# Corv/CUDA-GMM-MPI

Hardware: AMD Instinct MI355X
Metric: em_iterations_per_sec (higher is better)
Workload: dtype bf16; 1 GPU; model=gmm_em, n_events=1000000, events_per_gpu=1000000, dims=24, clusters=64, parallelism=dp1, device=cuda

## Files before the change

### cuda_gmm_mpi_amd/engine.py

```python
from __future__ import annotations

import dataclasses

import numpy as np
import torch

from .models.merge import HostClusters, reduce_order_batched
from .models.seed import seed_means_host, seed_state
from .models.state import GmmState
from .ops import functional as F
from .parallel import dist as pdist
from .utils.config import GmmConfig, em_epsilon, rissanen_score
from .utils.timers import Profile


@dataclasses.dataclass
class SweepResult:
    state: GmmState
    num_clusters: int
    min_rissanen: float
    likelihood: float
    rissanen_by_k: dict[int, float]


# ... 132 lines not shown
        st = self.state.shrink(k)
        empty_f = torch.empty(0, dtype=torch.float32, device=self.device)
        empty_b = torch.empty(0, dtype=torch.bfloat16, device=self.device)
        logdet = torch.empty(k, dtype=torch.float32, device=self.device)
        hip_ext().constants(st.R.contiguous(), st.means.contiguous(),
                            empty_f, st.Rinv, logdet, empty_f, empty_f,
                            empty_b, empty_f, False)

    def _sync_add(self, k: int) -> None:
        if self._add is not None:
            st = self.state.shrink(k)
            self._add[:k] = st.constant + torch.log(st.pi)


    def _estep(self, k: int, need_lik: bool = True) -> torch.Tensor | None:
        st = self.state.shrink(k)
        with self.profile.time("e_step"):
            self._w_is_logw = False
            if self.use_fused_estep and self.use_lds_estep:
                add = self._add[:k]
                if self.mfac32 is not None:
                    w, lik = F.estep_fused_f32_lds(self.x_estep,
                                                   self.mfac32[:k], add,
                                                   self.w[:k], need_lik)
                else:
                    w, lik = F.estep_fused_lds(self.x_estep, self.mfac[:k],
                                               add, self.w[:k], need_lik)
            elif self.use_fused_estep:
                self._w_is_logw = True
                add = self._add[:k]
                if self.mfac32 is not None:
                    w, lik = F.estep_fused_f32(self.x_estep, self.mfac32[:k],
                                               add, self.w[:k], self._lse,
                                               need_lik)
                else:
                    w, lik = F.estep_fused(self.x_estep, self.mfac[:k], add,
                                           self.w[:k], self._lse, need_lik)
            elif self.use_big_estep:
                add = self._add[:k]
                if self.mfac32 is not None:
                    logw = F.estep_logw_big_f32(self.x_estep,
                                                self.mfac32[:k], add,
                                                self.w[:k])
                    self._w_is_logw = True
                else:
                    logw = F.estep_logw_big(self.x_estep, self.mfac[:k],
                                            add, self.w[:k])
                lik = F.estep_lse(logw, self._lse, need_lik)
                self._w_is_logw = True
            elif self.device.type == "cuda":
                logw = F.estep_logw(
                    self.x_estep, st.means, st.Rinv, st.constant, st.pi,
                    self.cfg.diag_only, out=self.w[:k],
                )
                lik = F.estep_lse(logw, self._lse, need_lik)
                self._w_is_logw = True
            else:
                logw = F.estep_logw(
                    self.x_estep, st.means, st.Rinv, st.constant, st.pi,
                    self.cfg.diag_only, out=self.w[:k],
                )
                w, lik = F.estep_posteriors(logw)
        self.profile.count("regroup")
        return lik

    def _finish_likelihood(self, lik_part: torch.Tensor) -> None:
        with self.profile.time("comm"):
            t = lik_part.reshape(1)
            pdist.all_reduce_(t)
            self._lik_dev.copy_(t)

    def _reduce_likelihood(self, lik_part: torch.Tensor) -> float:
        self._finish_likelihood(lik_part)
        return float(self._lik_dev.item())

    def _iteration_body(self, k: int, need_lik: bool = True) -> None:
        self._mstep(k)
        lik = self._estep(k, need_lik)
        if need_lik and lik is not None:
            self._finish_likelihood(lik)

    def _can_graph(self) -> bool:
        import os
        if not self.use_graphs or os.environ.get("GMM_NO_GRAPHS"):
            return False
        if self.device.type != "cuda":
            return False
        if self.world > 1:
            return bool(os.environ.get("GMM_DIST_GRAPHS"))
        return True

    def _mstep(self, k: int) -> None:
        st = self.state.shrink(k)
# ... 378 lines not shown
```

### cuda_gmm_mpi_amd/ops/functional.py

```python
from __future__ import annotations

import os

import torch

from . import cpu_reference as cpu
from .backend import hip_ext


def estep_logw(x: torch.Tensor, means: torch.Tensor, rinv: torch.Tensor,
               constant: torch.Tensor, pi: torch.Tensor,
               diag_only: bool = False,
               out: torch.Tensor | None = None) -> torch.Tensor:
    if x.is_cuda:
        k, n = means.shape[0], x.shape[1]
        if out is None:
            out = torch.empty((k, n), dtype=torch.float32, device=x.device)
        hip_ext().estep_logw(
            x, means, rinv, constant, torch.log(pi), out, bool(diag_only)
        )
        return out
    logw = cpu.estep_logw(x.float(), means, rinv, constant, pi, diag_only)
    if out is not None:
        out.copy_(logw)
        return out
    return logw


def estep_posteriors(logw: torch.Tensor) -> tuple[torch.Tensor, torch.Tensor]:
    if logw.is_cuda:
        nblocks = 1024
        partial = torch.zeros(nblocks, dtype=torch.float32, device=logw.device)
        hip_ext().estep_posteriors(logw, partial)
        return logw, partial.sum()
    w, lik = cpu.estep_posteriors(logw)
    logw.copy_(w)
    return logw, lik


def estep_lse(logw: torch.Tensor, lse: torch.Tensor,
              need_lik: bool = True) -> torch.Tensor | None:
    nblocks = 1024
    partial = torch.zeros(nblocks, dtype=torch.float32, device=logw.device)
    hip_ext().estep_lse(logw, lse, partial)
    if not need_lik:
        return None
    lik = torch.empty(1, dtype=torch.float32, device=logw.device)
    hip_ext().reduce_scalar(partial, lik)
    return lik


def mstep_n_means(x_aug_t: torch.Tensor, w: torch.Tensor
                  ) -> tuple[torch.Tensor, torch.Tensor]:
    nm = w @ x_aug_t
    return nm[:, -1].contiguous(), nm[:, :-1].contiguous()


_tri_cache: dict = {}


def _tri_unpack_index(d: int, device) -> torch.Tensor:
    key = (d, str(device))
    idx = _tri_cache.get(key)
    if idx is None:
        full = torch.empty(d, d, dtype=torch.long)
        for i in range(d):
            for j in range(d):
                r, c = (i, j) if i >= j else (j, i)
                full[i, j] = r * (r + 1) // 2 + c
        idx = full.reshape(-1).to(device)
# ... 93 lines not shown
                if out is not None:
                    const_t.copy_(cval)
                else:
                    const_t = cval
                add_t.copy_(cval + torch.log(pi_t))
            return rinv, const_t
        hip_ext().constants(r, means, empty, rinv, logdet, empty, empty,
                            mfac, mfac32, bool(diag_only))
        const = -d * 0.5 * cpu.LOG_2PI - 0.5 * logdet
        if out is not None:
            out[1].copy_(const)
            const = out[1]
        return rinv, const
    rinv_c, const_c = cpu.compute_constants(r, diag_only)
    if out is not None:
        out[0].copy_(rinv_c)
        out[1].copy_(const_c)
        return out[0], out[1]
    return rinv_c, const_c


def _run_fused(entry: str, tile: int, z: torch.Tensor, fac: torch.Tensor,
               add: torch.Tensor, w_out: torch.Tensor, need_lik: bool,
               *lse: torch.Tensor) -> tuple[torch.Tensor, torch.Tensor | None]:
    ext = hip_ext()
    nblk = (z.shape[1] + tile - 1) // tile
    partial = torch.empty(nblk, dtype=torch.float32, device=z.device)
    getattr(ext, entry)(z, fac, add, w_out, *lse, partial)
    if not need_lik:
        return w_out, None
    lik = torch.empty(1, dtype=torch.float32, device=z.device)
    ext.reduce_scalar(partial, lik)
    return w_out, lik


def estep_fused(z: torch.Tensor, mfac: torch.Tensor, add: torch.Tensor,
                w_out: torch.Tensor, lse: torch.Tensor,
                need_lik: bool = True
                ) -> tuple[torch.Tensor, torch.Tensor | None]:
    return _run_fused("estep_fused", 256, z, mfac, add, w_out, need_lik, lse)


def estep_fused_available(device: torch.device, dtype: str, d: int,
                          k: int) -> bool:
    return device.type == "cuda" and d <= 31


def estep_fused_lds_available(device: torch.device, dtype: str, d: int,
                              k: int) -> bool:
    if device.type != "cuda" or d > 31:
        return False
    if dtype == "bf16":
        return 128 * 40 * 2 + 4 * k * 132 <= 64 * 1024
    return 4 * (128 * 33 + k * 132) <= 64 * 1024


def estep_fused_lds(z: torch.Tensor, mfac: torch.Tensor, add: torch.Tensor,
                    w_out: torch.Tensor, need_lik: bool = True
                    ) -> tuple[torch.Tensor, torch.Tensor | None]:
    legacy = os.environ.get("GMM_ESTEP_LDS", "lds2") == "legacy"
    return _run_fused("estep_fused_lds" if legacy else "estep_fused_lds2",
                      128, z, mfac, add, w_out, need_lik)


def estep_fused_f32_lds(z: torch.Tensor, mfac32: torch.Tensor,
                        add: torch.Tensor, w_out: torch.Tensor,
                        need_lik: bool = True
                        ) -> tuple[torch.Tensor, torch.Tensor | None]:
    return _run_fused("estep_fused_f32_lds", 128, z, mfac32, add, w_out,
                      need_lik)


def estep_fused_f32(z: torch.Tensor, mfac32: torch.Tensor, add: torch.Tensor,
                    w_out: torch.Tensor, lse: torch.Tensor,
                    need_lik: bool = True
                    ) -> tuple[torch.Tensor, torch.Tensor | None]:
    return _run_fused("estep_fused_f32", 256, z, mfac32, add, w_out,
                      need_lik, lse)


def estep_big_available(device: torch.device, dtype: str, d: int) -> bool:
    return device.type == "cuda" and dtype in ("bf16", "fp32") and 1 <= d <= 142


def mfac_shape(d: int) -> tuple[int, int, int]:
    rows = ((d + 31) // 32) * 32
    kc = (d + 1 + 15) // 16
    kct = 2 if kc <= 2 else 3 if kc == 3 else 5 if kc <= 5 else 9
    return 2, rows, kct * 16


def estep_logw_big(z: torch.Tensor, mfac: torch.Tensor, add: torch.Tensor,
                   out: torch.Tensor) -> torch.Tensor:
    hip_ext().estep_logw_big(z, mfac, add, out)
    return out


def estep_logw_big_f32(z: torch.Tensor, mfac32: torch.Tensor,
                       add: torch.Tensor, out: torch.Tensor) -> torch.Tensor:
    hip_ext().estep_logw_big_f32(z, mfac32, add, out)
    return out
# ... 92 lines not shown
```

### cuda_gmm_mpi_amd/ops/hip/estep_fused.hip

```cpp
#pragma once

#include "gmm_common.h"

namespace gmm {

struct FacB16 {
  using In = __hip_bfloat16;
  using Z = __bf16;
  static constexpr int ZROW = 40;
  static constexpr int CELLS = 2 * 32 * 32;

  bf16x8 h0, l0, h1, l1;
  float add;

  __device__ __forceinline__ void load(const In* mfac, const float* addv,
                                       int c, int j32, int g2) {
    const bf16x8* mf = (const bf16x8*)mfac;
    const int64_t base = ((int64_t)c * 2) * 32 * 4;
    h0 = mf[base + j32 * 4 + g2];
    l0 = mf[base + 32 * 4 + j32 * 4 + g2];
    h1 = mf[base + j32 * 4 + 2 + g2];
    l1 = mf[base + 32 * 4 + j32 * 4 + 2 + g2];
    add = addv[c];
  }
};

struct FacF32 {
  using In = float;
  using Z = float;
  static constexpr int ZROW = 33;
  static constexpr int CELLS = 32 * 32;
};

template <typename Fac, int BE>
constexpr int z_tile_floats() {
  return BE * Fac::ZROW * (int)sizeof(typename Fac::Z) / 4;
}

__device__ __forceinline__ float sqnorm(const f32x16_t& y) {
  float s = 0.0f;
#pragma unroll
  for (int r = 0; r < 16; ++r) s = fmaf(y[r], y[r], s);
  return s;
}

constexpr int EST_BE = 256;

template <typename Fac>
constexpr size_t est_lds_bytes() {
  return sizeof(float) *
         (z_tile_floats<Fac, EST_BE>() + (2 * (NT / WAVE) + 1) * EST_BE);
}

__global__ void __launch_bounds__(NT)
estep_fused_kernel(const __hip_bfloat16* __restrict__ z,
                   const __hip_bfloat16* __restrict__ mfac,
                   const float* __restrict__ add,
                   float* __restrict__ w_out, float* __restrict__ lse_out,
                   float* __restrict__ partial, int d, int k, int64_t n) {
  extern __shared__ float lds[];
  __hip_bfloat16* zs = (__hip_bfloat16*)lds;
  float* mstate = lds + (EST_BE * FacB16::ZROW) / 2;
  float* sstate = mstate + (NT / WAVE) * EST_BE;
  float* lse = sstate + (NT / WAVE) * EST_BE;

// ... 446 lines not shown
    const int t = threadIdx.x;
    float m = lw[t];
#pragma unroll 4
    for (int c = 1; c < k; ++c) m = fmaxf(m, lw[c * lrow + t]);
    float s = 0.0f;
#pragma unroll 4
    for (int c = 0; c < k; ++c) {
      const float e = __expf(lw[c * lrow + t] - m);
      lw[c * lrow + t] = e;
      s += e;
    }
    const float inv = 1.0f / s;
#pragma unroll 4
    for (int c = 0; c < k; ++c)
      w_out[(int64_t)c * n + e0 + t] = lw[c * lrow + t] * inv;
    acc = m + __logf(s);
  }
  __shared__ float wsum[NT / WAVE];
  block_sum(acc, wsum, partial);
}

constexpr int ESTL2_NS = 8;

__global__ void __launch_bounds__(NT, 3)
estep_fused_lds2_kernel(const __hip_bfloat16* __restrict__ z,
                        const __hip_bfloat16* __restrict__ mfac,
                        const float* __restrict__ add,
                        float* __restrict__ w_out,
                        float* __restrict__ partial, int d, int k, int64_t n,
                        int vec4) {
  extern __shared__ float lds[];
  constexpr int lrow = ESTL_LROW;
  constexpr int ZROW = FacB16::ZROW;
  __hip_bfloat16* zs = (__hip_bfloat16*)lds;
  float* lw = lds + z_tile_floats<FacB16, ESTL_BE>();

  const int wave = __builtin_amdgcn_readfirstlane(threadIdx.x / WAVE);
  const int lane = threadIdx.x & (WAVE - 1);
  const int64_t e0 = (int64_t)blockIdx.x * ESTL_BE;
  const int cnt = (int)min((int64_t)ESTL_BE, n - e0);

  {
    const unsigned short* zu = (const unsigned short*)z;
    const int e = threadIdx.x & (ESTL_BE - 1);
    const int o_lo = wave >> 1;
    unsigned short v[2][8];
// ... 40 lines not shown
  bf16x8 b0[ESTL_BE / 32], b1[ESTL_BE / 32];
#pragma unroll
  for (int t = 0; t < ESTL_BE / 32; ++t) {
    b0[t] = *(const bf16x8*)(zs + (t * 32 + j32) * ZROW + 8 * g2);
    b1[t] = *(const bf16x8*)(zs + (t * 32 + j32) * ZROW + 16 + 8 * g2);
  }
  auto cluster = [&](const FacB16& f, int c) {
    f32x16_t y[ESTL_BE / 32];
#pragma unroll
    for (int t = 0; t < ESTL_BE / 32; ++t)
      y[t] = __builtin_amdgcn_mfma_f32_32x32x16_bf16(
          f.h0, b0[t], (f32x16_t)(0.0f), 0, 0, 0);
#pragma unroll
    for (int t = 0; t < ESTL_BE / 32; ++t)
      y[t] = __builtin_amdgcn_mfma_f32_32x32x16_bf16(f.h1, b1[t], y[t], 0, 0, 0);
#pragma unroll
    for (int t = 0; t < ESTL_BE / 32; ++t)
      y[t] = __builtin_amdgcn_mfma_f32_32x32x16_bf16(f.l0, b0[t], y[t], 0, 0, 0);
#pragma unroll
    for (int t = 0; t < ESTL_BE / 32; ++t)
      y[t] = __builtin_amdgcn_mfma_f32_32x32x16_bf16(f.l1, b1[t], y[t], 0, 0, 0);
    float s[ESTL_BE / 32];
#pragma unroll
    for (int t = 0; t < ESTL_BE / 32; ++t) s[t] = sqnorm(y[t]);
#pragma unroll
    for (int t = 0; t < ESTL_BE / 32; t += 2) {
      const auto sw = __builtin_amdgcn_permlane32_swap(
          __float_as_uint(s[t]), __float_as_uint(s[t + 1]), false, false);
      const float st = __uint_as_float(sw[0]) + __uint_as_float(sw[1]);
      lw[c * lrow + (t + g2) * 32 + j32] = -0.5f * st + f.add;
    }
  };
  FacB16 fa, fb;
  int c = wave;
  fa.load(mfac, add, min(c, k - 1), j32, g2);
  for (; c + nwaves < k; c += 2 * nwaves) {
    fb.load(mfac, add, c + nwaves, j32, g2);
    __builtin_amdgcn_sched_barrier(0);
    cluster(fa, c);
    __builtin_amdgcn_sched_barrier(0);
    fa.load(mfac, add, min(c + 2 * nwaves, k - 1), j32, g2);
    __builtin_amdgcn_sched_barrier(0);
    cluster(fb, c + nwaves);
    __builtin_amdgcn_sched_barrier(0);
  }
  if (c < k) cluster(fa, c);
  __syncthreads();
// ... 90 lines not shown
```

### cuda_gmm_mpi_amd/ops/hip/gmm_ext.hip

```cpp
#include <ATen/hip/HIPContext.h>
#include <torch/extension.h>

#include <hip/hip_runtime.h>
#include <hip/hip_bf16.h>

#define HIP_CHECK(expr)                                                     \
  do {                                                                      \
    hipError_t _e = (expr);                                                 \
    TORCH_CHECK(_e == hipSuccess, "HIP error: ", hipGetErrorString(_e));    \
  } while (0)

#include "gmm_kernels.hip"

namespace {

constexpr int kNT = 256;

hipStream_t stream() { return at::hip::getCurrentHIPStream().stream(); }

void check_f32(const torch::Tensor& t, const char* name) {
  TORCH_CHECK(t.is_cuda() && t.is_contiguous() &&
                  t.scalar_type() == torch::kFloat32,
              name, " must be contiguous fp32 on device");
}
// ... 138 lines not shown
  else if (ppt <= 4) LAUNCH_COV(4);
  else if (ppt <= 8) LAUNCH_COV(8);
  else if (ppt <= 17) LAUNCH_COV(17);
  else if (ppt <= 33) LAUNCH_COV(33);
  else TORCH_CHECK(false, "D too large for covariance kernel (max 128)");
#undef LAUNCH_COV
  HIP_CHECK(hipGetLastError());
}

void mstep_covariance_partials(torch::Tensor x, torch::Tensor w,
                               torch::Tensor lse, torch::Tensor partials) {
  TORCH_CHECK(x.is_cuda() && x.is_contiguous(), "x must be contiguous device");
  check_f32(w, "w");
  check_f32(partials, "partials");
  if (x.scalar_type() == torch::kFloat32) {
    mstep_cov_impl<float>(x, w, lse, partials);
  } else if (x.scalar_type() == torch::kBFloat16) {
    mstep_cov_impl<__hip_bfloat16>(x, w, lse, partials);
  } else {
    TORCH_CHECK(false, "x must be fp32 or bf16");
  }
}

void constants(torch::Tensor r, torch::Tensor means, torch::Tensor pi,
               torch::Tensor rinv, torch::Tensor logdet,
               torch::Tensor constant, torch::Tensor add, torch::Tensor mfac,
               torch::Tensor mfac32, bool diag_only) {
  check_f32(r, "r");
  check_f32(means, "means");
  check_f32(rinv, "rinv");
  check_f32(logdet, "logdet");
  const int k = (int)r.size(0);
  const int d = (int)r.size(1);
  const bool make_mfac = mfac.numel() > 0;
  __hip_bfloat16* mp = nullptr;
  float* mp32 = nullptr;
  if (mfac32.numel() > 0) {
    TORCH_CHECK(mfac32.is_cuda() && mfac32.is_contiguous() &&
                    mfac32.scalar_type() == torch::kFloat32,
                "mfac32 must be contiguous fp32");
    mp32 = mfac32.data_ptr<float>();
  }
  if (make_mfac) {
    const int rows = gmm::mfac_rows(d);
    const int kct = gmm::mfac_kct(d);
    TORCH_CHECK(mfac.is_cuda() && mfac.is_contiguous() &&
                    mfac.scalar_type() == torch::kBFloat16 &&
                    mfac.numel() == (int64_t)k * 2 * rows * kct * 16 &&
                    d <= 142,
                "mfac must be bf16 [K,2,RT*32,KCT*16] with D <= 142");
    mp = reinterpret_cast<__hip_bfloat16*>(mfac.data_ptr());
  }
  auto s = stream();
  float* pip = pi.numel() > 0 ? pi.data_ptr<float>() : nullptr;
  float* cst = constant.numel() > 0 ? constant.data_ptr<float>() : nullptr;
  float* addp = add.numel() > 0 ? add.data_ptr<float>() : nullptr;
  TORCH_CHECK(addp == nullptr || pip != nullptr, "add output requires pi");
  if (diag_only) {
    hipLaunchKernelGGL(gmm::constants_diag_kernel, dim3(k), dim3(kNT), 0, s,
                       r.data_ptr<float>(), rinv.data_ptr<float>(),
                       logdet.data_ptr<float>(), d);
    if (make_mfac) {
      hipLaunchKernelGGL(gmm::emit_mfac_from_r_kernel, dim3(k), dim3(kNT),
                         sizeof(float) * (2 * (size_t)d * (d | 1) + d), s,
                         r.data_ptr<float>(), means.data_ptr<float>(), mp,
                         mp32, d, nullptr, nullptr, nullptr);
    }
  } else {
    const size_t lds = sizeof(float) * (2 * (size_t)d * (d | 1) + d);
    if (lds > 64 * 1024) {
      HIP_CHECK(hipFuncSetAttribute(
          reinterpret_cast<const void*>(&gmm::constants_lu_kernel),
          hipFuncAttributeMaxDynamicSharedMemorySize, (int)lds));
    }
// ... 225 lines not shown
void estep_fused_lds(torch::Tensor z, torch::Tensor mfac, torch::Tensor add,
                     torch::Tensor w_out, torch::Tensor partial) {
  launch_fused_lds<gmm::FacB16>("estep_fused_lds",
                                gmm::estep_fused_lds_kernel, z, mfac, add,
                                w_out, partial);
}

void estep_fused_f32_lds(torch::Tensor z, torch::Tensor mfac32,
                         torch::Tensor add, torch::Tensor w_out,
                         torch::Tensor partial) {
  launch_fused_lds<gmm::FacF32>("estep_fused_f32_lds",
                                gmm::estep_fused_f32_lds_kernel, z, mfac32,
                                add, w_out, partial);
}

void estep_fused_lds2(torch::Tensor z, torch::Tensor mfac, torch::Tensor add,
                      torch::Tensor w_out, torch::Tensor partial) {
  const char* name = "estep_fused_lds2";
  const FusedShape s = check_fused<gmm::FacB16>(name, z, mfac, add, w_out,
                                                partial, gmm::ESTL_BE);
  const int vec4 = s.n % 4 == 0 &&
                   reinterpret_cast<uintptr_t>(w_out.data_ptr()) % 16 == 0;
  const size_t lds = fused_lds_budget<gmm::FacB16>(name, s.k);
  hipLaunchKernelGGL(gmm::estep_fused_lds2_kernel, dim3((uint32_t)s.nblk),
                     dim3(kNT), lds, stream(), data_as<__hip_bfloat16>(z),
                     data_as<__hip_bfloat16>(mfac), add.data_ptr<float>(),
                     w_out.data_ptr<float>(), partial.data_ptr<float>(), s.d,
                     s.k, s.n, vec4);
  HIP_CHECK(hipGetLastError());
}

void estep_logw_big(torch::Tensor z, torch::Tensor mfac, torch::Tensor add,
                    torch::Tensor logw) {
  TORCH_CHECK(z.is_cuda() && z.is_contiguous() &&
                  z.scalar_type() == torch::kBFloat16,
              "z must be contiguous bf16 [D,N]");
  TORCH_CHECK(mfac.is_contiguous() && mfac.scalar_type() == torch::kBFloat16);
  check_f32(add, "add");
  check_f32(logw, "logw");
  const int d = (int)z.size(0);
  const int64_t n = z.size(1);
  const int k = (int)add.size(0);
  TORCH_CHECK(d >= 1 && d <= 142, "estep_logw_big supports D <= 143");
  TORCH_CHECK(logw.size(0) == k && logw.size(1) == n, "logw shape");
  const int kct = gmm::mfac_kct(d);
  const int rows = gmm::mfac_rows(d);
  const int rt_n = rows / 32;
  const int arow = kct * 16 + 8;
  const size_t lds256 = (size_t)(2 * rows + 256) * arow * 2 +
                        (size_t)rt_n * 256 * 4;
  const size_t lds128 = (size_t)(2 * rows + 128) * arow * 2 +
// ... 103 lines not shown
                     stream(), x.data_ptr<float>(), w.data_ptr<float>(),
                     lse_ptr(lse, n), partials.data_ptr<float>(), d, k, n,
                     nchunk);
  HIP_CHECK(hipGetLastError());
}

void mfma_probe32(torch::Tensor a, torch::Tensor b, torch::Tensor c) {
  TORCH_CHECK(a.scalar_type() == torch::kBFloat16 && a.numel() == 32 * 16);
  TORCH_CHECK(b.scalar_type() == torch::kBFloat16 && b.numel() == 16 * 32);
  check_f32(c, "c");
  hipLaunchKernelGGL(gmm::mfma_probe32_kernel, dim3(1), dim3(64), 0, stream(),
                     reinterpret_cast<const __hip_bfloat16*>(a.data_ptr()),
                     reinterpret_cast<const __hip_bfloat16*>(b.data_ptr()),
                     c.data_ptr<float>());
  HIP_CHECK(hipGetLastError());
}

void reduce_chunks(torch::Tensor partials, torch::Tensor out) {
  check_f32(partials, "partials");
  check_f32(out, "out");
  const int c = (int)partials.size(0);
  const int64_t m = partials.numel() / c;
  TORCH_CHECK(out.numel() == m, "out shape");
  const int grid = (int)std::min<int64_t>((m + kNT - 1) / kNT, 4096);
  hipLaunchKernelGGL(gmm::reduce_chunks_kernel, dim3(grid), dim3(kNT), 0,
                     stream(), partials.data_ptr<float>(),
                     out.data_ptr<float>(), c, m);
  HIP_CHECK(hipGetLastError());
}

void reduce_scalar(torch::Tensor in, torch::Tensor out) {
  check_f32(in, "in");
  check_f32(out, "out");
  TORCH_CHECK(out.numel() >= 1);
  hipLaunchKernelGGL(gmm::reduce_scalar_kernel, dim3(1), dim3(kNT), 0,
                     stream(), in.data_ptr<float>(), out.data_ptr<float>(),
                     in.numel());
  HIP_CHECK(hipGetLastError());
}

void mstep_finalize(torch::Tensor packed, torch::Tensor avgvar,
                    int64_t world, torch::Tensor n_out, torch::Tensor means,
                    torch::Tensor r_out, torch::Tensor pi, bool diag_only) {
  check_f32(packed, "packed");
  check_f32(avgvar, "avgvar");
  check_f32(n_out, "n_out");
  check_f32(means, "means");
  check_f32(r_out, "r_out");
// ... 20 lines not shown
                         torch::Tensor mfac32) {
  check_f32(packed, "packed");
  check_f32(avgvar, "avgvar");
  check_f32(n_out, "n_out");
  check_f32(means, "means");
  check_f32(r_out, "r_out");
  check_f32(pi, "pi");
  check_f32(constant, "constant");
  check_f32(add, "add");
  const int k = (int)means.size(0);
  const int d = (int)means.size(1);
  TORCH_CHECK(packed.size(0) == k &&
                  packed.size(1) == (d + 1) * (d + 2) / 2,
              "packed shape mismatch");
  TORCH_CHECK(mfac.numel() > 0 && mfac.scalar_type() == torch::kBFloat16 &&
              mfac.is_contiguous());
  __hip_bfloat16* mp =
      reinterpret_cast<__hip_bfloat16*>(mfac.data_ptr());
  float* mp32 = nullptr;
  if (mfac32.numel() > 0) {
    check_f32(mfac32, "mfac32");
    mp32 = mfac32.data_ptr<float>();
  }
  const size_t lds = sizeof(float) * (2 * (size_t)d * (d | 1) + d);
  if (lds > 64 * 1024) {
    HIP_CHECK(hipFuncSetAttribute(
        reinterpret_cast<const void*>(&gmm::mstep_finalize_emit_kernel),
        hipFuncAttributeMaxDynamicSharedMemorySize, (int)lds));
  }
  hipLaunchKernelGGL(gmm::mstep_finalize_emit_kernel, dim3(k), dim3(kNT),
                     lds, stream(), packed.data_ptr<float>(),
                     avgvar.data_ptr<float>(), (int)world,
                     n_out.data_ptr<float>(), means.data_ptr<float>(),
                     r_out.data_ptr<float>(), pi.data_ptr<float>(),
                     constant.data_ptr<float>(), add.data_ptr<float>(), mp,
                     mp32, d, k);
  HIP_CHECK(hipGetLastError());
}

void emit_factors(torch::Tensor r, torch::Tensor means,
                  torch::Tensor mfac, torch::Tensor mfac32,
                  torch::Tensor pi, torch::Tensor constant,
                  torch::Tensor add) {
  check_f32(r, "r");
  check_f32(means, "means");
  const int k = (int)r.size(0);
  const int d = (int)r.size(1);
  __hip_bfloat16* mp = nullptr;
  float* mp32 = nullptr;
  if (mfac.numel() > 0) {
    TORCH_CHECK(mfac.scalar_type() == torch::kBFloat16 && mfac.is_contiguous());
    mp = reinterpret_cast<__hip_bfloat16*>(mfac.data_ptr());
  }
  if (mfac32.numel() > 0) {
    check_f32(mfac32, "mfac32");
    mp32 = mfac32.data_ptr<float>();
  }
  const size_t lds = sizeof(float) * (2 * (size_t)d * (d | 1) + d);
  if (lds > 64 * 1024) {
    HIP_CHECK(hipFuncSetAttribute(
        reinterpret_cast<const void*>(&gmm::emit_mfac_from_r_kernel),
        hipFuncAttributeMaxDynamicSharedMemorySize, (int)lds));
  }
  const float* pip = pi.numel() > 0 ? pi.data_ptr<float>() : nullptr;
  float* cst = constant.numel() > 0 ? constant.data_ptr<float>() : nullptr;
  float* addp = add.numel() > 0 ? add.data_ptr<float>() : nullptr;
  TORCH_CHECK(addp == nullptr || pip != nullptr, "add output requires pi");
  hipLaunchKernelGGL(gmm::emit_mfac_from_r_kernel, dim3(k), dim3(kNT),
                     lds, stream(), r.data_ptr<float>(),
                     means.data_ptr<float>(), mp, mp32, d, pip, cst, addp);
  HIP_CHECK(hipGetLastError());
}

void mfma_probe(torch::Tensor a, torch::Tensor b, torch::Tensor c) {
  TORCH_CHECK(a.scalar_type() == torch::kBFloat16 && a.numel() == 16 * 32);
  TORCH_CHECK(b.scalar_type() == torch::kBFloat16 && b.numel() == 32 * 16);
  check_f32(c, "c");
  hipLaunchKernelGGL(gmm::mfma_probe_kernel, dim3(1), dim3(64), 0, stream(),
                     reinterpret_cast<const __hip_bfloat16*>(a.data_ptr()),
                     reinterpret_cast<const __hip_bfloat16*>(b.data_ptr()),
// ... 56 lines not shown
```

### cuda_gmm_mpi_amd/ops/hip/gmm_kernels.hip

```cpp
#include "gmm_common.h"

namespace gmm {

__device__ inline void tri_row_col(int t, int* i, int* j) {
  int r = (int)((sqrtf(8.0f * t + 1.0f) - 1.0f) * 0.5f);
  while ((r + 1) * (r + 2) / 2 <= t) ++r;
  while (r * (r + 1) / 2 > t) --r;
  *i = r;
  *j = t - r * (r + 1) / 2;
}

__device__ inline int mfma_b16_k(int group, int u) { return 8 * group + u; }

__host__ __device__ inline int kc_tier(int kc) {
  return kc <= 2 ? 2 : kc == 3 ? 3 : kc <= 5 ? 5 : 9;
}

__host__ __device__ inline int mfac_rows(int d) { return ((d + 31) / 32) * 32; }
__host__ __device__ inline int mfac_kct(int d) {
  return kc_tier((d + 1 + 15) / 16);
}

__device__ inline void stage_cluster_params(
    const float* __restrict__ means, const float* __restrict__ rinv,
// ... 152 lines not shown
    float s = 0.0f;
#pragma unroll 4
    for (int c = 0; c < k; ++c) s += __expf(logw[(int64_t)c * n + e] - m);
    const float denom = m + __logf(s);
    lse[e] = denom;
    acc += denom;
  }
  __shared__ float wsum[NT / WAVE];
  for (int off = WAVE / 2; off > 0; off >>= 1)
    acc += __shfl_down(acc, off, WAVE);
  const int wid = threadIdx.x / WAVE;
  if ((threadIdx.x & (WAVE - 1)) == 0) wsum[wid] = acc;
  __syncthreads();
  if (threadIdx.x == 0) {
    float total = 0.0f;
    for (int wv = 0; wv < NT / WAVE; ++wv) total += wsum[wv];
    partial[blockIdx.x] = total;
  }
}

__global__ void __launch_bounds__(NT)
reduce_chunks_kernel(const float* __restrict__ in, float* __restrict__ out,
                     int c, int64_t m) {
  for (int64_t j = (int64_t)blockIdx.x * NT + threadIdx.x; j < m;
       j += (int64_t)gridDim.x * NT) {
    float acc[8] = {0, 0, 0, 0, 0, 0, 0, 0};
    int i = 0;
    for (; i + 8 <= c; i += 8) {
#pragma unroll
      for (int u = 0; u < 8; ++u) acc[u] += in[(int64_t)(i + u) * m + j];
    }
    for (; i < c; ++i) acc[0] += in[(int64_t)i * m + j];
    out[j] = ((acc[0] + acc[1]) + (acc[2] + acc[3])) +
             ((acc[4] + acc[5]) + (acc[6] + acc[7]));
  }
}

__global__ void __launch_bounds__(NT)
reduce_scalar_kernel(const float* __restrict__ in, float* __restrict__ out,
                     int64_t n) {
  float acc = 0.0f;
  for (int64_t i = threadIdx.x; i < n; i += NT) acc += in[i];
  __shared__ float wsum[NT / WAVE];
  for (int off = WAVE / 2; off > 0; off >>= 1)
    acc += __shfl_down(acc, off, WAVE);
  if ((threadIdx.x & (WAVE - 1)) == 0) wsum[threadIdx.x / WAVE] = acc;
  __syncthreads();
  if (threadIdx.x == 0) {
    float total = 0.0f;
    for (int wv = 0; wv < NT / WAVE; ++wv) total += wsum[wv];
    out[0] = total;
  }
}

template <int PPT, typename T>
__global__ void __launch_bounds__(NT)
mstep_cov_kernel(const T* __restrict__ x, const float* __restrict__ w,
                 const float* __restrict__ lse,
                 float* __restrict__ partials, int d, int k, int64_t n,
                 int te, int nchunk) {
  extern __shared__ float lds[];
  const int row = te + 4;
  float* xs = lds;
  float* wt = lds + (int64_t)d * row;

// ... 94 lines not shown
    pi[c] = (n_c < 0.5f) ? 1e-10f : n_c / total;
  }
  for (int i = threadIdx.x; i < d; i += NT) {
    const float m = gt05 ? row[p + i] / n_c : 0.0f;
    mu[i] = m;
    means[(int64_t)c * d + i] = m;
  }
  __syncthreads();
  const float reg = world * avgvar[c];
  for (int t = threadIdx.x; t < p; t += NT) {
    int i, j;
    tri_row_col(t, &i, &j);
    float cov = ge1 ? row[t] - n_c * mu[i] * mu[j] : 0.0f;
    if (diag_only && i != j) cov = 0.0f;
    if (i == j) cov += reg;
    float rv;
    if (gt05) rv = cov / n_c;
    else rv = (i == j) ? 1.0f : 0.0f;
    r_out[((int64_t)c * d + i) * d + j] = rv;
    if (i != j) r_out[((int64_t)c * d + j) * d + i] = rv;
  }
}

__device__ inline void emit_mfac(float* a, float* o,
                                 const float* __restrict__ r_global,
                                 const float* __restrict__ means,
                                 __hip_bfloat16* __restrict__ mfac,
                                 float* __restrict__ mfac32, int c, int d,
                                 const float* __restrict__ pi = nullptr,
                                 float* __restrict__ constant = nullptr,
                                 float* __restrict__ add = nullptr) {
  const int tid = threadIdx.x;
  const int ldp = d | 1;
  float* u0 = o + d * ldp;
  for (int t = tid; t < d * d; t += blockDim.x)
    a[(t / d) * ldp + t % d] = r_global[(int64_t)c * d * d + t];
  __syncthreads();
  for (int j = 0; j < d; ++j) {
    if (tid == 0) {
      const float diag0 = fabsf(a[j * ldp + j]);
      float s = a[j * ldp + j];
      for (int kk = 0; kk < j; ++kk) s -= a[j * ldp + kk] * a[j * ldp + kk];
      a[j * ldp + j] = sqrtf(fmaxf(s, 1e-8f * diag0 + 1e-30f));
    }
    __syncthreads();
    const float piv = a[j * ldp + j];
    for (int i = j + 1 + tid; i < d; i += blockDim.x) {
      float s = a[i * ldp + j];
#pragma unroll 8
      for (int kk = 0; kk < j; ++kk) s -= a[i * ldp + kk] * a[j * ldp + kk];
      a[i * ldp + j] = s / piv;
    }
    __syncthreads();
  }
  if (constant != nullptr) {
    __shared__ float wsum_e[NT / WAVE];
    const int nw = (blockDim.x + WAVE - 1) / WAVE;
    float acc = 0.0f;
    for (int i = tid; i < d; i += blockDim.x)
      acc += __logf(a[i * ldp + i]);
    for (int off = WAVE / 2; off > 0; off >>= 1)
      acc += __shfl_down(acc, off, WAVE);
    if ((tid & (WAVE - 1)) == 0) wsum_e[tid / WAVE] = acc;
    __syncthreads();
    if (tid == 0) {
      const float ld2 = 2.0f * (wsum_e[0] + ((nw > 1) ? wsum_e[1] : 0.0f) +
                                ((nw > 2) ? wsum_e[2] : 0.0f) +
                                ((nw > 3) ? wsum_e[3] : 0.0f));
      const float cst = -d * 0.5f * 1.8378770664093453f - 0.5f * ld2;
      constant[c] = cst;
      if (add) add[c] = cst + __logf(pi[c]);
    }
    __syncthreads();
  }
  for (int t = tid; t < d * ldp; t += blockDim.x) o[t] = a[t];
  __syncthreads();
  for (int i = tid; i < d; i += blockDim.x) {
    for (int j = i; j < d; ++j) {
      float xv = 1.0f;
      if (i != j) {
        xv = 0.0f;
#pragma unroll 8
        for (int kk = i; kk < j; ++kk)
          xv -= o[j * ldp + kk] * a[kk * ldp + i];
      }
      a[j * ldp + i] = xv / o[j * ldp + j];
    }
  }
  __syncthreads();
  for (int i = tid; i < d; i += blockDim.x) {
    float s = 0.0f;
#pragma unroll 8
    for (int j = 0; j <= i; ++j) s += a[i * ldp + j] * means[c * d + j];
    u0[i] = -s;
  }
  __syncthreads();
  const int rows = mfac_rows(d);
  const int cols = mfac_kct(d) * 16;
  const int cells = rows * cols;
  __hip_bfloat16* out = mfac + (int64_t)c * 2 * cells;
  float* out32 = mfac32 ? mfac32 + (int64_t)c * cells : nullptr;
  for (int t = tid; t < cells; t += blockDim.x) {
    const int i = t / cols, kx = t % cols;
    float v = 0.0f;
    if (i < d) {
      if (kx < d) v = (kx <= i) ? a[i * ldp + kx] : 0.0f;
      else if (kx == d) v = u0[i];
    }
    const __hip_bfloat16 hi = __float2bfloat16(v);
    out[t] = hi;
    out[cells + t] = __float2bfloat16(v - __bfloat162float(hi));
    if (out32) out32[t] = v;
  }
}

__global__ void __launch_bounds__(NT)
mstep_finalize_emit_kernel(const float* __restrict__ packed,
                           const float* __restrict__ avgvar, int world,
                           float* __restrict__ n_out,
                           float* __restrict__ means,
                           float* __restrict__ r_out,
                           float* __restrict__ pi,
                           float* __restrict__ constant,
                           float* __restrict__ add,
                           __hip_bfloat16* __restrict__ mfac,
                           float* __restrict__ mfac32, int d, int k) {
  extern __shared__ float lds[];
  const int ldp = d | 1;
  float* a = lds;
  float* o = a + d * ldp;
  float* mu = o + d * ldp;
  const int c = blockIdx.x;
  const int dp = d + 1;
  const int pp = dp * (dp + 1) / 2;
  const int p = d * (d + 1) / 2;
  const float* row = packed + (int64_t)c * pp;
  const float n_c = row[pp - 1];
  const bool ge1 = n_c >= 1.0f;
  const bool gt05 = n_c > 0.5f;

  if (threadIdx.x == 0) {
    n_out[c] = n_c;
    float total = 0.0f;
    for (int cc = 0; cc < k; ++cc) total += packed[(int64_t)cc * pp + pp - 1];
    pi[c] = (n_c < 0.5f) ? 1e-10f : n_c / total;
  }
  for (int i = threadIdx.x; i < d; i += NT) {
    const float m = gt05 ? row[p + i] / n_c : 0.0f;
    mu[i] = m;
    means[(int64_t)c * d + i] = m;
  }
  __syncthreads();
  const float reg = world * avgvar[c];
  for (int t = threadIdx.x; t < p; t += NT) {
    int i, j;
    tri_row_col(t, &i, &j);
    float cov = ge1 ? row[t] - n_c * mu[i] * mu[j] : 0.0f;
    if (i == j) cov += reg;
    float rv;
    if (gt05) rv = cov / n_c;
    else rv = (i == j) ? 1.0f : 0.0f;
    r_out[((int64_t)c * d + i) * d + j] = rv;
    if (i != j) r_out[((int64_t)c * d + j) * d + i] = rv;
  }
  __syncthreads();
  emit_mfac(a, o, r_out, means, mfac, mfac32, c, d, pi, constant, add);
}

__global__ void __launch_bounds__(NT)
constants_lu_kernel(const float* __restrict__ r,
                    const float* __restrict__ means,
                    const float* __restrict__ pi, float* __restrict__ rinv,
                    float* __restrict__ logdet,
                    float* __restrict__ constant, float* __restrict__ add,
                    __hip_bfloat16* __restrict__ mfac,
                    float* __restrict__ mfac32, int d) {
  extern __shared__ float a[];
  const int c = blockIdx.x;
  const int tid = threadIdx.x;
  const int ldp = d | 1;
  float* o = a + d * ldp;
  const float* rc = r + (int64_t)c * d * d;
  float* oc = rinv + (int64_t)c * d * d;

  for (int t = tid; t < d * d; t += blockDim.x)
    a[(t / d) * ldp + t % d] = rc[t];
  __syncthreads();

  if (d == 1) {
// ... 1294 lines not shown
```

Before: 2349 iters/s.

## Streamline factor emission, templatize E-step sqnorm, and tune reductions

Several unrelated changes land together. The E-step lds2 kernel is templated on the number of live accumulator rows, so the squared-norm sums only the rows that matter for small D. The M-step finalize Cholesky and inverse are rewritten as row-per-thread loops with fewer barriers, the covariance is written directly into LDS instead of being re-read from global memory, and the factor output is emitted with vectorized stores. Smaller edits unroll the chunk and scalar reductions, use a wave-wide sum for cluster totals, and write the likelihood straight into a persistent buffer to skip a copy. These trim per-iteration overhead in small kernels but change floating-point rounding order.

```diff
diff --git a/cuda_gmm_mpi_amd/engine.py b/cuda_gmm_mpi_amd/engine.py
--- a/cuda_gmm_mpi_amd/engine.py
+++ b/cuda_gmm_mpi_amd/engine.py
@@ -178,20 +178,24 @@
                 if self.mfac32 is not None:
                     w, lik = F.estep_fused_f32_lds(self.x_estep,
                                                    self.mfac32[:k], add,
-                                                   self.w[:k], need_lik)
+                                                   self.w[:k], need_lik,
+                                                   lik_out=self._lik_dev)
                 else:
                     w, lik = F.estep_fused_lds(self.x_estep, self.mfac[:k],
-                                               add, self.w[:k], need_lik)
+                                               add, self.w[:k], need_lik,
+                                               lik_out=self._lik_dev)
             elif self.use_fused_estep:
                 self._w_is_logw = True
                 add = self._add[:k]
                 if self.mfac32 is not None:
                     w, lik = F.estep_fused_f32(self.x_estep, self.mfac32[:k],
                                                add, self.w[:k], self._lse,
-                                               need_lik)
+                                               need_lik,
+                                               lik_out=self._lik_dev)
                 else:
                     w, lik = F.estep_fused(self.x_estep, self.mfac[:k], add,
-                                           self.w[:k], self._lse, need_lik)
+                                           self.w[:k], self._lse, need_lik,
+                                           lik_out=self._lik_dev)
             elif self.use_big_estep:
                 add = self._add[:k]
                 if self.mfac32 is not None:
@@ -202,14 +206,16 @@
                 else:
                     logw = F.estep_logw_big(self.x_estep, self.mfac[:k],
                                             add, self.w[:k])
-                lik = F.estep_lse(logw, self._lse, need_lik)
+                lik = F.estep_lse(logw, self._lse, need_lik,
+                                  lik_out=self._lik_dev)
                 self._w_is_logw = True
             elif self.device.type == "cuda":
                 logw = F.estep_logw(
                     self.x_estep, st.means, st.Rinv, st.constant, st.pi,
                     self.cfg.diag_only, out=self.w[:k],
                 )
-                lik = F.estep_lse(logw, self._lse, need_lik)
+                lik = F.estep_lse(logw, self._lse, need_lik,
+                                  lik_out=self._lik_dev)
                 self._w_is_logw = True
             else:
                 logw = F.estep_logw(
@@ -224,7 +230,8 @@
         with self.profile.time("comm"):
             t = lik_part.reshape(1)
             pdist.all_reduce_(t)
-            self._lik_dev.copy_(t)
+            if t.data_ptr() != self._lik_dev.data_ptr():
+                self._lik_dev.copy_(t)
 
     def _reduce_likelihood(self, lik_part: torch.Tensor) -> float:
         self._finish_likelihood(lik_part)
diff --git a/cuda_gmm_mpi_amd/ops/functional.py b/cuda_gmm_mpi_amd/ops/functional.py
--- a/cuda_gmm_mpi_amd/ops/functional.py
+++ b/cuda_gmm_mpi_amd/ops/functional.py
@@ -39,13 +39,15 @@
 
 
 def estep_lse(logw: torch.Tensor, lse: torch.Tensor,
-              need_lik: bool = True) -> torch.Tensor | None:
+              need_lik: bool = True,
+              lik_out: torch.Tensor | None = None) -> torch.Tensor | None:
     nblocks = 1024
     partial = torch.zeros(nblocks, dtype=torch.float32, device=logw.device)
     hip_ext().estep_lse(logw, lse, partial)
     if not need_lik:
         return None
-    lik = torch.empty(1, dtype=torch.float32, device=logw.device)
+    lik = (lik_out if lik_out is not None
+           else torch.empty(1, dtype=torch.float32, device=logw.device))
     hip_ext().reduce_scalar(partial, lik)
     return lik
 
@@ -185,23 +187,26 @@
 
 def _run_fused(entry: str, tile: int, z: torch.Tensor, fac: torch.Tensor,
                add: torch.Tensor, w_out: torch.Tensor, need_lik: bool,
-               *lse: torch.Tensor) -> tuple[torch.Tensor, torch.Tensor | None]:
+               *lse: torch.Tensor, lik_out: torch.Tensor | None = None
+               ) -> tuple[torch.Tensor, torch.Tensor | None]:
     ext = hip_ext()
     nblk = (z.shape[1] + tile - 1) // tile
     partial = torch.empty(nblk, dtype=torch.float32, device=z.device)
     getattr(ext, entry)(z, fac, add, w_out, *lse, partial)
     if not need_lik:
         return w_out, None
-    lik = torch.empty(1, dtype=torch.float32, device=z.device)
+    lik = (lik_out if lik_out is not None
+           else torch.empty(1, dtype=torch.float32, device=z.device))
     ext.reduce_scalar(partial, lik)
     return w_out, lik
 
 
 def estep_fused(z: torch.Tensor, mfac: torch.Tensor, add: torch.Tensor,
                 w_out: torch.Tensor, lse: torch.Tensor,
-                need_lik: bool = True
+                need_lik: bool = True, lik_out: torch.Tensor | None = None
                 ) -> tuple[torch.Tensor, torch.Tensor | None]:
-    return _run_fused("estep_fused", 256, z, mfac, add, w_out, need_lik, lse)
+    return _run_fused("estep_fused", 256, z, mfac, add, w_out, need_lik, lse,
+                      lik_out=lik_out)
 
 
 def estep_fused_available(device: torch.device, dtype: str, d: int,
@@ -219,27 +224,30 @@
 
 
 def estep_fused_lds(z: torch.Tensor, mfac: torch.Tensor, add: torch.Tensor,
-                    w_out: torch.Tensor, need_lik: bool = True
+                    w_out: torch.Tensor, need_lik: bool = True,
+                    lik_out: torch.Tensor | None = None
                     ) -> tuple[torch.Tensor, torch.Tensor | None]:
     legacy = os.environ.get("GMM_ESTEP_LDS", "lds2") == "legacy"
     return _run_fused("estep_fused_lds" if legacy else "estep_fused_lds2",
-                      128, z, mfac, add, w_out, need_lik)
+                      128, z, mfac, add, w_out, need_lik, lik_out=lik_out)
 
 
 def estep_fused_f32_lds(z: torch.Tensor, mfac32: torch.Tensor,
                         add: torch.Tensor, w_out: torch.Tensor,
-                        need_lik: bool = True
+                        need_lik: bool = True,
+                        lik_out: torch.Tensor | None = None
                         ) -> tuple[torch.Tensor, torch.Tensor | None]:
     return _run_fused("estep_fused_f32_lds", 128, z, mfac32, add, w_out,
-                      need_lik)
+                      need_lik, lik_out=lik_out)
 
 
 def estep_fused_f32(z: torch.Tensor, mfac32: torch.Tensor, add: torch.Tensor,
                     w_out: torch.Tensor, lse: torch.Tensor,
-                    need_lik: bool = True
+                    need_lik: bool = True,
+                    lik_out: torch.Tensor | None = None
                     ) -> tuple[torch.Tensor, torch.Tensor | None]:
     return _run_fused("estep_fused_f32", 256, z, mfac32, add, w_out,
-                      need_lik, lse)
+                      need_lik, lse, lik_out=lik_out)
 
 
 def estep_big_available(device: torch.device, dtype: str, d: int) -> bool:
diff --git a/cuda_gmm_mpi_amd/ops/hip/estep_fused.hip b/cuda_gmm_mpi_amd/ops/hip/estep_fused.hip
--- a/cuda_gmm_mpi_amd/ops/hip/estep_fused.hip
+++ b/cuda_gmm_mpi_amd/ops/hip/estep_fused.hip
@@ -37,10 +37,11 @@
   return BE * Fac::ZROW * (int)sizeof(typename Fac::Z) / 4;
 }
 
+template <int NL>
 __device__ __forceinline__ float sqnorm(const f32x16_t& y) {
   float s = 0.0f;
 #pragma unroll
-  for (int r = 0; r < 16; ++r) s = fmaf(y[r], y[r], s);
+  for (int r = 0; r < NL; ++r) s = fmaf(y[r], y[r], s);
   return s;
 }
 
@@ -533,6 +534,7 @@
 
 constexpr int ESTL2_NS = 8;
 
+template <int NL>
 __global__ void __launch_bounds__(NT, 3)
 estep_fused_lds2_kernel(const __hip_bfloat16* __restrict__ z,
                         const __hip_bfloat16* __restrict__ mfac,
@@ -619,7 +621,7 @@
       y[t] = __builtin_amdgcn_mfma_f32_32x32x16_bf16(f.l1, b1[t], y[t], 0, 0, 0);
     float s[ESTL_BE / 32];
 #pragma unroll
-    for (int t = 0; t < ESTL_BE / 32; ++t) s[t] = sqnorm(y[t]);
+    for (int t = 0; t < ESTL_BE / 32; ++t) s[t] = sqnorm<NL>(y[t]);
 #pragma unroll
     for (int t = 0; t < ESTL_BE / 32; t += 2) {
       const auto sw = __builtin_amdgcn_permlane32_swap(
diff --git a/cuda_gmm_mpi_amd/ops/hip/gmm_ext.hip b/cuda_gmm_mpi_amd/ops/hip/gmm_ext.hip
--- a/cuda_gmm_mpi_amd/ops/hip/gmm_ext.hip
+++ b/cuda_gmm_mpi_amd/ops/hip/gmm_ext.hip
@@ -184,6 +184,17 @@
   }
 }
 
+void check_factor_out(const torch::Tensor& mfac, const torch::Tensor& mfac32,
+                      int d) {
+  TORCH_CHECK(d <= kNT, "factor emission needs D <= ", kNT);
+  TORCH_CHECK(mfac.numel() == 0 ||
+                  reinterpret_cast<uintptr_t>(mfac.data_ptr()) % 16 == 0,
+              "mfac must be 16-byte aligned");
+  TORCH_CHECK(mfac32.numel() == 0 ||
+                  reinterpret_cast<uintptr_t>(mfac32.data_ptr()) % 16 == 0,
+              "mfac32 must be 16-byte aligned");
+}
+
 void constants(torch::Tensor r, torch::Tensor means, torch::Tensor pi,
                torch::Tensor rinv, torch::Tensor logdet,
                torch::Tensor constant, torch::Tensor add, torch::Tensor mfac,
@@ -212,6 +223,7 @@
                     d <= 142,
                 "mfac must be bf16 [K,2,RT*32,KCT*16] with D <= 142");
     mp = reinterpret_cast<__hip_bfloat16*>(mfac.data_ptr());
+    check_factor_out(mfac, mfac32, d);
   }
   auto s = stream();
   float* pip = pi.numel() > 0 ? pi.data_ptr<float>() : nullptr;
@@ -483,11 +495,18 @@
   const int vec4 = s.n % 4 == 0 &&
                    reinterpret_cast<uintptr_t>(w_out.data_ptr()) % 16 == 0;
   const size_t lds = fused_lds_budget<gmm::FacB16>(name, s.k);
-  hipLaunchKernelGGL(gmm::estep_fused_lds2_kernel, dim3((uint32_t)s.nblk),
-                     dim3(kNT), lds, stream(), data_as<__hip_bfloat16>(z),
-                     data_as<__hip_bfloat16>(mfac), add.data_ptr<float>(),
-                     w_out.data_ptr<float>(), partial.data_ptr<float>(), s.d,
-                     s.k, s.n, vec4);
+#define LAUNCH_LDS2(NL)                                                      \
+  hipLaunchKernelGGL(gmm::estep_fused_lds2_kernel<NL>,                       \
+                     dim3((uint32_t)s.nblk), dim3(kNT), lds, stream(),       \
+                     data_as<__hip_bfloat16>(z),                             \
+                     data_as<__hip_bfloat16>(mfac), add.data_ptr<float>(),   \
+                     w_out.data_ptr<float>(), partial.data_ptr<float>(),     \
+                     s.d, s.k, s.n, vec4)
+  if (s.d <= 8) LAUNCH_LDS2(4);
+  else if (s.d <= 16) LAUNCH_LDS2(8);
+  else if (s.d <= 24) LAUNCH_LDS2(12);
+  else LAUNCH_LDS2(16);
+#undef LAUNCH_LDS2
   HIP_CHECK(hipGetLastError());
 }
 
@@ -637,8 +656,9 @@
   const int c = (int)partials.size(0);
   const int64_t m = partials.numel() / c;
   TORCH_CHECK(out.numel() == m, "out shape");
-  const int grid = (int)std::min<int64_t>((m + kNT - 1) / kNT, 4096);
-  hipLaunchKernelGGL(gmm::reduce_chunks_kernel, dim3(grid), dim3(kNT), 0,
+  constexpr int kRcNT = 64;
+  const int grid = (int)std::min<int64_t>((m + kRcNT - 1) / kRcNT, 8192);
+  hipLaunchKernelGGL(gmm::reduce_chunks_kernel, dim3(grid), dim3(kRcNT), 0,
                      stream(), partials.data_ptr<float>(),
                      out.data_ptr<float>(), c, m);
   HIP_CHECK(hipGetLastError());
@@ -705,6 +725,7 @@
     check_f32(mfac32, "mfac32");
     mp32 = mfac32.data_ptr<float>();
   }
+  check_factor_out(mfac, mfac32, d);
   const size_t lds = sizeof(float) * (2 * (size_t)d * (d | 1) + d);
   if (lds > 64 * 1024) {
     HIP_CHECK(hipFuncSetAttribute(
@@ -739,6 +760,7 @@
     check_f32(mfac32, "mfac32");
     mp32 = mfac32.data_ptr<float>();
   }
+  check_factor_out(mfac, mfac32, d);
   const size_t lds = sizeof(float) * (2 * (size_t)d * (d | 1) + d);
   if (lds > 64 * 1024) {
     HIP_CHECK(hipFuncSetAttribute(
diff --git a/cuda_gmm_mpi_amd/ops/hip/gmm_kernels.hip b/cuda_gmm_mpi_amd/ops/hip/gmm_kernels.hip
--- a/cuda_gmm_mpi_amd/ops/hip/gmm_kernels.hip
+++ b/cuda_gmm_mpi_amd/ops/hip/gmm_kernels.hip
@@ -198,10 +198,19 @@
 __global__ void __launch_bounds__(NT)
 reduce_chunks_kernel(const float* __restrict__ in, float* __restrict__ out,
                      int c, int64_t m) {
-  for (int64_t j = (int64_t)blockIdx.x * NT + threadIdx.x; j < m;
-       j += (int64_t)gridDim.x * NT) {
+  for (int64_t j = (int64_t)blockIdx.x * blockDim.x + threadIdx.x; j < m;
+       j += (int64_t)gridDim.x * blockDim.x) {
     float acc[8] = {0, 0, 0, 0, 0, 0, 0, 0};
     int i = 0;
+    for (; i + 32 <= c; i += 32) {
+      float v[32];
+#pragma unroll
+      for (int u = 0; u < 32; ++u) v[u] = in[(int64_t)(i + u) * m + j];
+#pragma unroll
+      for (int q = 0; q < 4; ++q)
+#pragma unroll
+        for (int u = 0; u < 8; ++u) acc[u] += v[8 * q + u];
+    }
     for (; i + 8 <= c; i += 8) {
 #pragma unroll
       for (int u = 0; u < 8; ++u) acc[u] += in[(int64_t)(i + u) * m + j];
@@ -215,8 +224,19 @@
 __global__ void __launch_bounds__(NT)
 reduce_scalar_kernel(const float* __restrict__ in, float* __restrict__ out,
                      int64_t n) {
+  constexpr int U = 16;
   float acc = 0.0f;
-  for (int64_t i = threadIdx.x; i < n; i += NT) acc += in[i];
+  for (int64_t i = threadIdx.x; i < n; i += (int64_t)U * NT) {
+    float v[U];
+#pragma unroll
+    for (int u = 0; u < U; ++u) {
+      const int64_t idx = i + (int64_t)u * NT;
+      v[u] = in[idx < n ? idx : i];
+    }
+#pragma unroll
+    for (int u = 0; u < U; ++u)
+      if (i + (int64_t)u * NT < n) acc += v[u];
+  }
   __shared__ float wsum[NT / WAVE];
   for (int off = WAVE / 2; off > 0; off >>= 1)
     acc += __shfl_down(acc, off, WAVE);
@@ -357,6 +377,12 @@
   }
 }
 
+__device__ __forceinline__ float unfused_mulsub(float acc, float x, float y) {
+  float p = x * y;
+  asm("" : "+v"(p));
+  return acc - p;
+}
+
 __device__ inline void emit_mfac(float* a, float* o,
                                  const float* __restrict__ r_global,
                                  const float* __restrict__ means,
@@ -368,25 +394,35 @@
   const int tid = threadIdx.x;
   const int ldp = d | 1;
   float* u0 = o + d * ldp;
-  for (int t = tid; t < d * d; t += blockDim.x)
-    a[(t / d) * ldp + t % d] = r_global[(int64_t)c * d * d + t];
-  __syncthreads();
-  for (int j = 0; j < d; ++j) {
-    if (tid == 0) {
-      const float diag0 = fabsf(a[j * ldp + j]);
-      float s = a[j * ldp + j];
-      for (int kk = 0; kk < j; ++kk) s -= a[j * ldp + kk] * a[j * ldp + kk];
-      a[j * ldp + j] = sqrtf(fmaxf(s, 1e-8f * diag0 + 1e-30f));
-    }
+  if (r_global != nullptr) {
+    for (int t = tid; t < d * d; t += blockDim.x)
+      a[(t / d) * ldp + t % d] = r_global[(int64_t)c * d * d + t];
     __syncthreads();
-    const float piv = a[j * ldp + j];
-    for (int i = j + 1 + tid; i < d; i += blockDim.x) {
-      float s = a[i * ldp + j];
+  }
+  {
+    const bool own = tid < d;
+    float* ri = a + tid * ldp;
+    float sd = 0.0f, diag0 = 0.0f;
+    if (own) {
+      sd = ri[tid];
+      diag0 = fabsf(sd);
+    }
+    if (tid == 0) ri[0] = sqrtf(fmaxf(sd, fmaf(1e-8f, diag0, 1e-30f)));
+    __syncthreads();
+    for (int j = 0; j + 1 < d; ++j) {
+      if (own && tid > j) {
+        const float* rj = a + j * ldp;
+        float s = ri[j];
 #pragma unroll 8
-      for (int kk = 0; kk < j; ++kk) s -= a[i * ldp + kk] * a[j * ldp + kk];
-      a[i * ldp + j] = s / piv;
-    }
-    __syncthreads();
+        for (int kk = 0; kk < j; ++kk) s = fmaf(-ri[kk], rj[kk], s);
+        const float l = s / rj[j];
+        ri[j] = l;
+        sd = fmaf(-l, l, sd);
+        if (tid == j + 1)
+          ri[tid] = sqrtf(fmaxf(sd, fmaf(1e-8f, diag0, 1e-30f)));
+      }
+      __syncthreads();
+    }
   }
   if (constant != nullptr) {
     __shared__ float wsum_e[NT / WAVE];
@@ -408,44 +444,80 @@
     }
     __syncthreads();
   }
-  for (int t = tid; t < d * ldp; t += blockDim.x) o[t] = a[t];
-  __syncthreads();
-  for (int i = tid; i < d; i += blockDim.x) {
+  if (tid < d) {
+    const int i = tid;
     for (int j = i; j < d; ++j) {
+      const float* lj = a + j * ldp;
       float xv = 1.0f;
       if (i != j) {
         xv = 0.0f;
-#pragma unroll 8
-        for (int kk = i; kk < j; ++kk)
-          xv -= o[j * ldp + kk] * a[kk * ldp + i];
-      }
-      a[j * ldp + i] = xv / o[j * ldp + j];
-    }
-  }
-  __syncthreads();
-  for (int i = tid; i < d; i += blockDim.x) {
+        int kk = i;
+        for (const int head = i + ((j - i) & 7); kk < head; ++kk)
+          xv = fmaf(-lj[kk], o[kk * ldp + i], xv);
+        for (; kk < j; kk += 8) {
+          float lv[8], fv[8];
+#pragma unroll
+          for (int u = 0; u < 8; ++u) {
+            lv[u] = lj[kk + u];
+            fv[u] = o[(kk + u) * ldp + i];
+          }
+#pragma unroll
+          for (int u = 0; u < 8; ++u) xv = unfused_mulsub(xv, lv[u], fv[u]);
+        }
+      }
+      o[j * ldp + i] = xv / lj[j];
+    }
+  }
+  __syncthreads();
+  if (tid < d) {
+    const float* fi = o + tid * ldp;
     float s = 0.0f;
 #pragma unroll 8
-    for (int j = 0; j <= i; ++j) s += a[i * ldp + j] * means[c * d + j];
-    u0[i] = -s;
+    for (int j = 0; j <= tid; ++j) s = fmaf(fi[j], means[c * d + j], s);
+    u0[tid] = -s;
   }
   __syncthreads();
   const int rows = mfac_rows(d);
   const int cols = mfac_kct(d) * 16;
   const int cells = rows * cols;
+  const int cpr = cols >> 3;
   __hip_bfloat16* out = mfac + (int64_t)c * 2 * cells;
   float* out32 = mfac32 ? mfac32 + (int64_t)c * cells : nullptr;
-  for (int t = tid; t < cells; t += blockDim.x) {
-    const int i = t / cols, kx = t % cols;
-    float v = 0.0f;
-    if (i < d) {
-      if (kx < d) v = (kx <= i) ? a[i * ldp + kx] : 0.0f;
-      else if (kx == d) v = u0[i];
-    }
-    const __hip_bfloat16 hi = __float2bfloat16(v);
-    out[t] = hi;
-    out[cells + t] = __float2bfloat16(v - __bfloat162float(hi));
-    if (out32) out32[t] = v;
+  for (int g = tid; g < rows * cpr; g += blockDim.x) {
+    const int i = g / cpr, kx0 = (g - i * cpr) << 3;
+    float v[8];
+#pragma unroll
+    for (int u = 0; u < 8; ++u) v[u] = 0.0f;
+    if (i < d && kx0 <= d) {
+      const float* fi = o + i * ldp;
+      const float ui = u0[i];
+#pragma unroll
+      for (int u = 0; u < 8; ++u) {
+        const int kx = kx0 + u;
+        const float f = fi[min(kx, i)];
+        v[u] = (kx <= i) ? f : ((kx == d) ? ui : 0.0f);
+      }
+    }
+    unsigned int ph[4], pl[4];
+#pragma unroll
+    for (int u = 0; u < 8; u += 2) {
+      const __hip_bfloat16 h0 = __float2bfloat16(v[u]);
+      const __hip_bfloat16 h1 = __float2bfloat16(v[u + 1]);
+      const __hip_bfloat16 l0 = __float2bfloat16(v[u] - __bfloat162float(h0));
+      const __hip_bfloat16 l1 =
+          __float2bfloat16(v[u + 1] - __bfloat162float(h1));
+      ph[u >> 1] = (unsigned int)__bfloat16_as_ushort(h0) |
+                   ((unsigned int)__bfloat16_as_ushort(h1) << 16);
+      pl[u >> 1] = (unsigned int)__bfloat16_as_ushort(l0) |
+                   ((unsigned int)__bfloat16_as_ushort(l1) << 16);
+    }
+    const int t = g << 3;
+    *(uint4*)(out + t) = make_uint4(ph[0], ph[1], ph[2], ph[3]);
+    *(uint4*)(out + cells + t) = make_uint4(pl[0], pl[1], pl[2], pl[3]);
+    if (out32) {
+      *(float4*)(out32 + t) = make_float4(v[0], v[1], v[2], v[3]);
+      *(float4*)(out32 + t + 4) = make_float4(v[4], v[5], v[6], v[7]);
+    }
   }
 }
 
@@ -474,11 +546,25 @@
   const bool ge1 = n_c >= 1.0f;
   const bool gt05 = n_c > 0.5f;
 
-  if (threadIdx.x == 0) {
-    n_out[c] = n_c;
+  if (threadIdx.x < WAVE) {
     float total = 0.0f;
-    for (int cc = 0; cc < k; ++cc) total += packed[(int64_t)cc * pp + pp - 1];
-    pi[c] = (n_c < 0.5f) ? 1e-10f : n_c / total;
+    for (int base = 0; base < k; base += WAVE) {
+      const int cc = min(base + (int)threadIdx.x, k - 1);
+      const int nv = __float_as_int(packed[(int64_t)cc * pp + pp - 1]);
+      const int cnt = min(WAVE, k - base);
+      if (cnt == WAVE) {
+#pragma unroll
+        for (int l = 0; l < WAVE; ++l)
+          total += __int_as_float(__builtin_amdgcn_readlane(nv, l));
+      } else {
+        for (int l = 0; l < cnt; ++l)
+          total += __int_as_float(__builtin_amdgcn_readlane(nv, l));
+      }
+    }
+    if (threadIdx.x == 0) {
+      n_out[c] = n_c;
+      pi[c] = (n_c < 0.5f) ? 1e-10f : n_c / total;
+    }
   }
   for (int i = threadIdx.x; i < d; i += NT) {
     const float m = gt05 ? row[p + i] / n_c : 0.0f;
@@ -490,16 +576,17 @@
   for (int t = threadIdx.x; t < p; t += NT) {
     int i, j;
     tri_row_col(t, &i, &j);
-    float cov = ge1 ? row[t] - n_c * mu[i] * mu[j] : 0.0f;
+    float cov = ge1 ? fmaf(-(n_c * mu[i]), mu[j], row[t]) : 0.0f;
     if (i == j) cov += reg;
     float rv;
     if (gt05) rv = cov / n_c;
     else rv = (i == j) ? 1.0f : 0.0f;
     r_out[((int64_t)c * d + i) * d + j] = rv;
     if (i != j) r_out[((int64_t)c * d + j) * d + i] = rv;
-  }
-  __syncthreads();
-  emit_mfac(a, o, r_out, means, mfac, mfac32, c, d, pi, constant, add);
+    a[i * ldp + j] = rv;
+  }
+  __syncthreads();
+  emit_mfac(a, o, nullptr, means, mfac, mfac32, c, d, pi, constant, add);
 }
 
 __global__ void __launch_bounds__(NT)
```

Measured after the change: 2574 iters/s, median of 6. +9.6%, better.
